# aloe101/GNOT-Replication

Measured on AMD Instinct MI355X. Metric: mesh points/sec (GNOT fwd+bwd, whole node), higher is better.
Workload: dtype fp32; 1 GPU; configs[2]: synthetic 3-D mesh of 262,144 points, d=256, 8 experts, 8 heads, 1 input function (805 points), fp32 fwd+bwd; samples_per_gpu=1, input_function_points=805, hidden=256, experts=8, heads=8, blocks=4, mlp_layers=4, input_functions=1, geometry=fixed, moe_recompute=False, parallelism=single, step=pack+fwd+RelL2+bwd+AdamW (native loss, native flat AdamW) (hipGraph replay)

## Files before the change

### gnot-replication_amd/csrc/engine.cpp

```cpp
#include <hip/hip_runtime.h>

#include <algorithm>
#include <cmath>
#include <cstdio>
#include <cstdlib>
#include <cstring>
#include <map>
#include <string>
#include <vector>

#include "../../include/gnot_hip.h"
#include "gnot_kernels.h"

namespace gnot {

static thread_local std::string g_err;

static int fail(int code, const std::string& msg) {
  g_err = msg;
  return code;
}

#define GNOT_CK(expr)                                                                           \
  do {                                                                                          \
// ... 487 lines not shown
      Img t = img(DT, DT);
      job(li, t, 0, 0, DT, DT, 1, -1, x6, li != io);
      p->T_img[li] = t;
    }
    if (!selftype)
      for (size_t i = 0; i < ik.size(); ++i)
        for (int li : {ik[i], iv[i]}) {
          Img t = new_img(DT, DT);
          job(li, t, 0, 0, DT, DT, 1, -1, 0, true);
          p->T_img[li] = t;
        }
  };
  for (int l = 0; l < p->L; ++l) {
    std::vector<int> ck, cv;
    for (int i = 0; i < p->KI; ++i) { ck.push_back(p->lin_ck(l, i)); cv.push_back(p->lin_cv(l, i)); }
    attn_imgs(p->cross_img[l], p->lin_cq(l), p->lin_co(l), ck, cv, p->I == 0);
    attn_imgs(p->self_img[l], p->lin_sq(l), p->lin_so(l), {p->lin_sk(l)}, {p->lin_sv(l)}, true);
    for (int e = 0; e < p->E; ++e) {
      chain_imgs(p->lin_f1(l, e, 0), DT, DT);
      chain_imgs(p->lin_f2(l, e, 0), DT, DT);
    }
  }
  chain_imgs(p->lin_out(0), DT, kt_of(p->out));
  p->pack_prefix.clear();
  int acc = 0;
  for (auto& J : p->pack_jobs) {
    p->pack_prefix.push_back(acc);
    acc += pack_tiles(J);
  }
  p->pack_tiles = acc;
}

constexpr long kWide128Wgs = 128;
static bool balanced_wgrad(const WgradGroup& G) {
  if (G.jobs.size() < 2) return false;
  for (const auto& J : G.jobs)
    if (J.P <= 0) return false;
  return 256 % (long)G.jobs.size() != 0;
}
static void finish_group(gnot_plan* p, WgradGroup& G) {
  G.x6 = true;
  for (const auto& J : G.jobs)
    if (J.w != nullptr || J.state_dh > 0 || J.diag_only) G.x6 = false;
  constexpr long x6_wgs = 256;
  const bool small = p->P < gnot_plan::kWgradSerialPoints;
  const long wide_wgs = !small ? 256 : p->npk() == 1 ? 64 : 128;
  const long w128_wgs = small && p->npk() != 1 ? 192 : kWide128Wgs;
  G.wide = G.x6 && p->D == 256 && !G.jobs.empty();
  for (const auto& J : G.jobs)
    if (J.out > 256 || J.in > 256) G.wide = false;
  G.tw = 256;
  if (G.x6 && !G.wide && p->D <= 128 && !G.jobs.empty()) {
    bool fits = true;
    for (const auto& J : G.jobs)
      if (J.out > 128 || J.in > 128) fits = false;
    if (fits) { G.wide = true; G.tw = 128; }
  }
  if (G.b16) G.wide = true;
  const long target = G.wide ? (G.tw == 128 ? w128_wgs : wide_wgs) : G.x6 ? x6_wgs : kTargetWGs;
  long tiles = 0;
  for (auto& J : G.jobs) {
    J.tiles_o = (J.out + kPTile - 1) / kPTile;
    J.tiles_i = (J.in + kPTile - 1) / kPTile;
    tiles += G.wide ? 1 : J.diag_only ? J.tiles_o : J.tiles_o * J.tiles_i;
  }
  const long want = std::max<long>(1, target / std::max<long>(tiles, 1));
  G.wg_prefix.clear();
  G.red_prefix.clear();
  G.segs.clear();
  G.seg_start.clear();
  G.slab_floats = 0;
  if (G.wide && G.tw == 256 && balanced_wgrad(G)) {
    long T = 0, maxrow = 1;
    for (const auto& J : G.jobs) {
      T += J.P;
      maxrow = std::max<long>(maxrow, G.b16 ? 512L : 4L * std::max<long>(std::max<long>(J.lddz, J.ldx), 1));
    }
    long C = std::max<long>((T + target - 1) / target, kMinSplitPoints);
    C = (C + 31) / 32 * 32;
    C = std::min<long>(C, ((1L << 31) - 1) / maxrow - 64);
    std::vector<long> jstart(G.jobs.size() + 1, 0);
    for (size_t j = 0; j < G.jobs.size(); ++j) jstart[j + 1] = jstart[j] + G.jobs[j].P;
    std::vector<int> nslots(G.jobs.size(), 0);
    size_t jj = 0;
    for (long w0 = 0; w0 < T; w0 += C) {
      const long w1 = std::min(T, w0 + C);
      G.seg_start.push_back((int)G.segs.size());
      while (jj < G.jobs.size() && jstart[jj + 1] <= w0) ++jj;
      for (size_t j = jj; j < G.jobs.size() && jstart[j] < w1; ++j) {
        const long b = std::max(w0, jstart[j]) - jstart[j], e = std::min(w1, jstart[j + 1]) - jstart[j];
        if (e > b) G.segs.push_back(int4{(int)j, nslots[j]++, (int)b, (int)e});
      }
    }
    G.seg_start.push_back((int)G.segs.size());
    int red = 0;
    for (size_t j = 0; j < G.jobs.size(); ++j) {
      auto& J = G.jobs[j];
      J.splits = std::max(1, nslots[j]);
      const int nt = J.tiles_o * J.tiles_i;
      J.slab_off = (long)G.slab_floats;
      G.slab_floats += (size_t)J.splits * nt * kPTile * (kPTile + 1);
      G.wg_prefix.push_back(0);
      G.red_prefix.push_back(red);
      red += nt * kPTile * (kPTile + 1);
    }
// ... 1653 lines not shown
```

### gnot-replication_amd/csrc/microbench.cpp

```cpp
#include <hip/hip_runtime.h>

#include <cstdio>
#include <algorithm>
#include <cmath>
#include <cstdlib>
#include <vector>

#include "gnot_kernels.h"

using namespace gnot;
#ifdef GNOT_DIAG_STAMP
namespace gnot {
hipError_t set_chain2_diag(int v);
}
#endif

#define CK(x)                                                                                   \
  do {                                                                                          \
    hipError_t e_ = (x);                                                                        \
    if (e_ != hipSuccess) {                                                                     \
      std::fprintf(stderr, "%s:%d %s -> %s\n", __FILE__, __LINE__, #x, hipGetErrorString(e_)); \
      std::exit(1);                                                                             \
    }                                                                                           \
  } while (0)

static float* dalloc(size_t n, float scale) {
  std::vector<float> h(n);
  for (size_t i = 0; i < n; ++i) h[i] = scale * ((float)((i * 2654435761u) % 2001) / 1000.0f - 1.0f);
  float* d = nullptr;
  CK(hipMalloc(&d, n * sizeof(float)));
  CK(hipMemcpy(d, h.data(), n * sizeof(float), hipMemcpyHostToDevice));
  return d;
}

template <typename F>
static double time_us(F&& f, int reps = 50) {
  hipEvent_t a, b;
  CK(hipEventCreate(&a));
  CK(hipEventCreate(&b));
  for (int i = 0; i < 5; ++i) f();
  CK(hipEventRecord(a, nullptr));
  for (int i = 0; i < reps; ++i) f();
  CK(hipEventRecord(b, nullptr));
  CK(hipEventSynchronize(b));
  float ms = 0.f;
  CK(hipEventElapsedTime(&ms, a, b));
  return ms * 1e3 / reps;
}

#ifdef GNOT_DIAG_STAMP
static void stamp_report(const char* name, ChainArgs a, bool bwd) {
  static unsigned long long* dbg = nullptr;
  const size_t n = (size_t)65536 * 8 * 3;
  if (!dbg) CK(hipMalloc(&dbg, n * sizeof(unsigned long long)));
  CK(hipMemset(dbg, 0, n * sizeof(unsigned long long)));
  a.dbg = dbg;
  CK(bwd ? launch_chain_bwd(a, nullptr) : launch_chain_fwd(a, nullptr));
  CK(hipDeviceSynchronize());
  std::vector<unsigned long long> h(n);
  CK(hipMemcpy(h.data(), dbg, n * sizeof(unsigned long long), hipMemcpyDeviceToHost));
  double body = 0, sync = 0, cnt = 0, waves = 0;
  for (size_t i = 0; i < n; i += 3)
    if (h[i + 2]) { body += (double)h[i]; sync += (double)h[i + 1]; cnt += (double)h[i + 2]; waves += 1; }
  std::printf("stamp %-28s waves %8.0f  syncs/wave %6.1f  sync share %5.3f  ticks/sync %7.1f  body ticks/interval %8.1f\n",
              name, waves, cnt / std::max(waves, 1.0), sync / std::max(body + sync, 1.0), sync / std::max(cnt, 1.0),
              body / std::max(cnt - waves, 1.0));
}
#define STAMP(name, args, bwd) stamp_report(name, args, bwd)
#else
#define STAMP(name, args, bwd) (void)0
#endif

int main(int argc, char** argv) {
  const int P = argc > 1 ? std::atoi(argv[1]) : 10000;
  const int D = argc > 2 ? std::atoi(argv[2]) : 128;
  const int E = argc > 3 ? std::atoi(argv[3]) : 4, NL = 5, DT = D / 16;
  const size_t img4 = (size_t)DT * ((DT + 1) / 2) * 3 * 64;
  float4* W = reinterpret_cast<float4*>(dalloc(img4 * 4 * NL * E * 2, 0.05f));
  float* bias = dalloc((size_t)NL * E * D, 0.01f);
  std::vector<ChainLayer> layers;
  for (int e = 0; e < E; ++e)
    for (int j = 0; j < NL; ++j) {
      const size_t k = (size_t)e * NL + j;
      layers.push_back(ChainLayer{W + 2 * k * img4, W + (2 * k + 1) * img4, bias + k * D});
    }
  ChainLayer* dlayers = nullptr;
  CK(hipMalloc(&dlayers, layers.size() * sizeof(ChainLayer)));
  CK(hipMemcpy(dlayers, layers.data(), layers.size() * sizeof(ChainLayer), hipMemcpyHostToDevice));
  float* X = dalloc((size_t)P * D, 1.0f);
  float* Y = dalloc((size_t)E * P * D, 0.0f);
  float* save = dalloc((size_t)E * NL * P * D, 1.0f);
  float* dz = dalloc((size_t)E * NL * P * D, 0.0f);
  float* scores = dalloc((size_t)P * 16, 0.25f);
  float* dscore = dalloc((size_t)P * 16, 0.0f);
  float* dX = dalloc((size_t)E * P * D, 0.0f);

  ChainArgs a{};
  a.D = D; a.KT0 = DT; a.OTL = DT; a.nlin = NL; a.in_dim = D; a.out_dim = D; a.P = P; a.nchains = E;
  a.layers = dlayers; a.X = X; a.ldx = D; a.Y = Y; a.ldy = D; a.y_chain_stride = (long)P * D;
  a.scores = scores; a.ldsc = 16; a.mode = CH_MOE;
  a.save = save; a.save_layer_stride = (long)P * D; a.save_chain_stride = (long)NL * P * D;
  const double fl = 2.0 * E * P * NL * (double)D * D;
  double t = time_us([&] { CK(launch_moe_combine(X, Y, (long)P * D, E, dX, (long)P * D, nullptr)); });
  std::printf("moe_combine E=%d P=%d D=%d: %8.2f us  %6.0f GB/s\n", E, P, D, t, (E + 2.0) * P * D * 4 / t / 1e3);
  t = time_us([&] { CK(launch_chain_fwd(a, nullptr)); });
  std::printf("chain_fwd  MoE E=%d P=%d D=%d: %8.2f us  %6.1f TFLOP/s\n", E, P, D, t, fl / t / 1e6);
  STAMP("chain_fwd MoE x6", a, false);
  {
    ChainArgs an = a;
    an.save = nullptr;
    t = time_us([&] { CK(launch_chain_fwd(an, nullptr)); });
    std::printf("chain_fwd  MoE no-save E=%d P=%d D=%d: %8.2f us  %6.1f TFLOP/s\n", E, P, D, t, fl / t / 1e6);
  }
  ChainArgs bw = a;
  bw.dY = X; bw.lddy = D; bw.dscore = dscore; bw.dz = dz; bw.dz_layer_stride = (long)P * D;
  bw.dz_chain_stride = (long)NL * P * D; bw.dX = dX; bw.lddx = D; bw.dx_chain_stride = (long)P * D;
  t = time_us([&] { CK(launch_chain_bwd(bw, nullptr)); });
  std::printf("chain_bwd  MoE E=%d P=%d D=%d: %8.2f us  %6.1f TFLOP/s\n", E, P, D, t, fl / t / 1e6);
  STAMP("chain_bwd MoE x6", bw, true);
  if (D == 256) {
    ChainArgs a1 = a, b1 = bw;
    a1.np = 1; b1.np = 1;
    t = time_us([&] { CK(launch_chain_fwd(a1, nullptr)); });
// ... 23 lines not shown
      t = time_us([&] { CK(launch_chain_bwd(bw, nullptr)); });
      std::printf("diag %d  fp32 (x6)    fwd %8.2f us  bwd %8.2f us\n", dg, tx, t);
    }
    CK(set_chain2_diag(0));
#else
    t = time_us([&] { CK(launch_chain_fwd(a3, nullptr)); });
    std::printf("chain_fwd  b16s stage E=%d P=%d D=%d: %8.2f us  %6.1f TFLOP/s\n", E, P, D, t, fl / t / 1e6);
    t = time_us([&] { CK(launch_chain_bwd(b3, nullptr)); });
    std::printf("chain_bwd  b16s stage E=%d P=%d D=%d: %8.2f us  %6.1f TFLOP/s\n", E, P, D, t, fl / t / 1e6);
#endif
  }

  if (argc > 4 && std::atoi(argv[4]) == 1) return 0;
  for (int NO : {D, 3 * D}) {
    LinearArgs l{};
    l.nseg = 1; l.X[0] = X; l.Wp[0] = W; l.ldx = D; l.nsum = 1; l.K = D; l.bias = bias; l.Y = Y; l.ldy = NO;
    l.NO = NO; l.P = P; l.epi = EPI_STORE; l.nsoft = 0; l.dh = 16;
    t = time_us([&] { CK(D == 256 ? launch_linear2(l, nullptr) : launch_linear(l, D, nullptr)); });
    std::printf("linear     P=%d K=%d NO=%d: %8.2f us  %6.1f TFLOP/s\n", P, D, NO, t, 2.0 * P * D * NO / t / 1e6);
    if (D == 256) {
      l.np = 1;
      t = time_us([&] { CK(launch_linear2(l, nullptr)); });
      std::printf("linear     P=%d K=%d NO=%d bf16: %8.2f us  %6.1f TFLOP/s\n", P, D, NO, t, 2.0 * P * D * NO / t / 1e6);
      l.np = 3;
    }
    if (D == 256 && NO == D) {
      l.epi = EPI_ACCUM;
      t = time_us([&] { CK(launch_linear2(l, nullptr)); });
      std::printf("linear     P=%d K=%d NO=%d accum: %8.2f us  %6.1f TFLOP/s\n", P, D, NO, t, 2.0 * P * D * NO / t / 1e6);
      l.nseg = 3; l.X[1] = X; l.X[2] = X; l.Wp[1] = W; l.Wp[2] = W; l.bias = nullptr;
      t = time_us([&] { CK(launch_linear2(l, nullptr)); });
      std::printf("linear     P=%d K=3x%d NO=%d accum: %8.2f us  %6.1f TFLOP/s\n", P, D, NO, t, 6.0 * P * D * NO / t / 1e6);
    }
  }
  {
    float* fresh = dalloc((size_t)E * NL * P * D, 0.5f);
    CK(hipMemcpy(dz, fresh, (size_t)E * NL * P * D * 4, hipMemcpyDeviceToDevice));
    CK(hipFree(fresh));
    fresh = dalloc((size_t)E * NL * P * D, 2.0f);
    CK(hipMemcpy(save, fresh, (size_t)E * NL * P * D * 4, hipMemcpyDeviceToDevice));
    CK(hipFree(fresh));
  }
  {
    std::vector<WgradJob> jobs;
    std::vector<int> wg_pre, red_pre;
    int wg = 0, red = 0;
    long slab_off = 0;
    float* dW = dalloc((size_t)E * NL * (D * D + D), 0.f);
    const int njobs = E * NL;
    const int tiles = ((D + 127) / 128) * ((D + 127) / 128);
    const long want = std::max<long>(1, 512 / ((long)njobs * tiles));
    for (int k = 0; k < njobs; ++k) {
      WgradJob J{};
      J.dz = dz + (size_t)k * P * D; J.lddz = D; J.x = save + (size_t)k * P * D; J.ldx = D; J.x_gelu = 1;
      J.out = D; J.in = D; J.dW = dW + (size_t)k * (D * D + D); J.db = J.dW + D * D; J.P = P;
      J.tiles_o = (D + 127) / 128; J.tiles_i = J.tiles_o;
      J.splits = (int)std::min<long>(std::min<long>(want, std::max<long>(1, P / 128)), 256);
      J.slab_off = slab_off;
      slab_off += (long)J.splits * tiles * 128 * 129;
      wg_pre.push_back(wg); wg += tiles * J.splits;
      red_pre.push_back(red); red += tiles * 128 * 129;
      jobs.push_back(J);
    }
    WgradJob* djobs = nullptr;
    int* dpre = nullptr;
    CK(hipMalloc(&djobs, jobs.size() * sizeof(WgradJob)));
// ... 14 lines not shown
    CK(hipMemcpy(got.data(), dW, ndw * 4, hipMemcpyDeviceToHost));
    double num = 0, den = 0;
    for (size_t i = 0; i < ndw; ++i) { num += (got[i] - ref[i]) * (double)(got[i] - ref[i]); den += (double)ref[i] * ref[i]; }
    std::printf("wgrad MoE  bf16x6:                     %8.2f us  %6.1f TFLOP/s  (rel-L2 vs fp32 %.2e)\n", t, fl / t / 1e6,
                std::sqrt(num / (den + 1e-30)));
    if (D == 256) {
      for (int wgs : {256, 512}) {
        std::vector<WgradJob> wj(jobs);
        std::vector<int> wpre;
        long soff = 0;
        const int splits = std::max(1, wgs / njobs);
        for (int k = 0; k < njobs; ++k) {
          wj[k].splits = splits;
          wj[k].slab_off = soff;
          soff += (long)splits * tiles * 128 * 129;
          wpre.push_back(k * splits);
        }
        wpre.insert(wpre.end(), red_pre.begin(), red_pre.end());
        WgradJob* dwj = nullptr;
        int* dwpre = nullptr;
        float* wslab = nullptr;
        CK(hipMalloc(&dwj, wj.size() * sizeof(WgradJob)));
        CK(hipMemcpy(dwj, wj.data(), wj.size() * sizeof(WgradJob), hipMemcpyHostToDevice));
        CK(hipMalloc(&dwpre, wpre.size() * sizeof(int)));
        CK(hipMemcpy(dwpre, wpre.data(), wpre.size() * sizeof(int), hipMemcpyHostToDevice));
        CK(hipMalloc(&wslab, soff * sizeof(float)));
        t = time_us([&] { CK(launch_wgrad(dwj, dwpre, njobs, njobs * splits, dwpre + njobs, red, wslab, nullptr, true, true)); }, 20);
        CK(hipDeviceSynchronize());
        CK(hipMemcpy(got.data(), dW, ndw * 4, hipMemcpyDeviceToHost));
        double n2 = 0, d2 = 0;
        for (size_t i = 0; i < ndw; ++i) { n2 += (got[i] - ref[i]) * (double)(got[i] - ref[i]); d2 += (double)ref[i] * ref[i]; }
        std::printf("wgrad MoE  bf16x6 wide 256x256 (%d WGs):  %8.2f us  %6.1f TFLOP/s  (rel-L2 vs fp32 %.2e)\n",
                    njobs * splits, t, fl / t / 1e6, std::sqrt(n2 / (d2 + 1e-30)));
        t = time_us([&] { CK(launch_wgrad(dwj, dwpre, njobs, njobs * splits, dwpre + njobs, red, wslab, nullptr, true, true, 1)); }, 20);
        CK(hipDeviceSynchronize());
        CK(hipMemcpy(got.data(), dW, ndw * 4, hipMemcpyDeviceToHost));
        n2 = 0; d2 = 0;
        for (size_t i = 0; i < ndw; ++i) { n2 += (got[i] - ref[i]) * (double)(got[i] - ref[i]); d2 += (double)ref[i] * ref[i]; }
        std::printf("wgrad MoE  bf16 wide 256x256 (%d WGs):    %8.2f us  %6.1f TFLOP/s  (rel-L2 vs fp32 %.2e)\n",
                    njobs * splits, t, fl / t / 1e6, std::sqrt(n2 / (d2 + 1e-30)));
        if (wgs == 512) {
          const char* what[3] = {"no-GELU operand", "L2-resident rows", "no-GELU + L2 rows"};
          for (int v = 0; v < 3; ++v) {
            std::vector<WgradJob> dj(wj);
            for (auto& J : dj) {
              if (v != 1) J.x_gelu = 0;
              if (v != 0) { J.lddz = 0; J.ldx = 0; }
            }
            CK(hipMemcpy(dwj, dj.data(), dj.size() * sizeof(WgradJob), hipMemcpyHostToDevice));
            t = time_us([&] { CK(launch_wgrad(dwj, dwpre, njobs, njobs * splits, dwpre + njobs, red, wslab, nullptr, true, true)); }, 20);
            std::printf("wgrad MoE  bf16x6 wide, %-18s   %8.2f us  %6.1f TFLOP/s\n", what[v], t, fl / t / 1e6);
          }
        }
        CK(hipFree(dwj));
        CK(hipFree(dwpre));
        CK(hipFree(wslab));
      }
    }
    {
      std::vector<WgradJob> ng(jobs);
      for (auto& J : ng) J.x_gelu = 0;
      WgradJob* dng = nullptr;
      CK(hipMalloc(&dng, ng.size() * sizeof(WgradJob)));
      CK(hipMemcpy(dng, ng.data(), ng.size() * sizeof(WgradJob), hipMemcpyHostToDevice));
      t = time_us([&] { CK(launch_wgrad(dng, dpre, njobs, wg, dpre + njobs, red, slab, nullptr)); }, 20);
      std::printf("wgrad MoE  no-GELU operand:            %8.2f us  %6.1f TFLOP/s\n", t, fl / t / 1e6);
// ... 55 lines not shown
```

### gnot-replication_amd/csrc/wgrad.hip

```cpp
#include <cstdlib>
#include <type_traits>

#include "gnot_common.h"
#include "gnot_kernels.h"
#include "x6_core.h"

namespace gnot {

typedef float f32x16 __attribute__((ext_vector_type(16)));

constexpr int kTile = 128;
constexpr int kStage = 32;
constexpr int kLdsRow = kTile;

GNOT_DEV int find_job(const int* __restrict__ prefix, int njobs, int idx) {
  int lo = 0, hi = njobs - 1;
  while (lo < hi) {
    const int mid = (lo + hi + 1) >> 1;
    if (prefix[mid] <= idx) lo = mid; else hi = mid - 1;
  }
  return lo;
}

struct StageRegs {
// ... 265 lines not shown
      asm volatile("" ::: "memory");
    }
  }

  const int ntile = J.tiles_o * J.tiles_i;
  const int tile = to * J.tiles_i + ti;
  float* S = slab + J.slab_off + ((long)split * ntile + tile) * (kTile * (kTile + 1));
#pragma unroll
  for (int a = 0; a < 2; ++a)
#pragma unroll
    for (int b = 0; b < 2; ++b)
#pragma unroll
      for (int r = 0; r < 16; ++r) {
        const int row = wo * 64 + a * 32 + (r & 3) + 8 * (r >> 2) + 4 * h;
        const int col = wi * 64 + b * 32 + r32;
        S[row * (kTile + 1) + col] = acc[a][b][r];
      }
  if (want_db) {
    __syncthreads();
    float* red = reinterpret_cast<float*>(lds);
    red[o * kTile + 2 * fp] = dbacc[0];
    red[o * kTile + 2 * fp + 1] = dbacc[1];
    __syncthreads();
    if (tid < kTile) S[tid * (kTile + 1) + kTile] = (red[tid] + red[kTile + tid]) + (red[2 * kTile + tid] + red[3 * kTile + tid]);
  }
}

constexpr int kWStage = 16;
constexpr int kWThreads = 512;
constexpr int w_threads(int tw) { return tw * 2; }
constexpr int w_piece(int tw) { return tw / 32 * 64; }
constexpr int w_buf(int np, int tw = 256) { return 2 * np * w_piece(tw); }
constexpr int kWRawSlot = 2 * 2 * 64;
constexpr int kWRawSlots = 2;
constexpr size_t w_lds_bytes(int np, int tw = 256) {
  return (2 * (size_t)w_buf(np, tw) + (size_t)(tw / 32) * kWRawSlots * kWRawSlot) * 16;
}

template <int OFF>
GNOT_DEV float lds_read_b32_off(unsigned addr) {
  float v;
  asm volatile("ds_read_b32 %0, %1 offset:%2" : "=v"(v) : "v"(addr), "n"(OFF) : "memory");
  return v;
}

template <int NP = 3, int TW = 256>
__global__ void __launch_bounds__(w_threads(TW)) pgemm_x6w_kernel(const WgradJob* __restrict__ jobs,
                                                                 const int* __restrict__ prefix, int njobs,
                                                                 float* __restrict__ slab,
                                                                 const int4* __restrict__ segs,
                                                                 const int* __restrict__ seg_start) {
  constexpr int NW = TW / 32;
  constexpr int FG = TW / 64;
  constexpr int WC = NW / 2;
  constexpr int RB = TW / 64;
  constexpr int kWPiece = w_piece(TW);
  extern __shared__ __attribute__((aligned(16))) u32x4 wl[];
  const int tid = threadIdx.x;
  const int lane = tid & 63, wave = __builtin_amdgcn_readfirstlane(tid >> 6);
  int k0 = 0, k1 = 1;
  if (segs != nullptr) { k0 = seg_start[blockIdx.x]; k1 = seg_start[blockIdx.x + 1]; }
  for (int kseg = k0; kseg < k1; ++kseg) {
  int j, split;
  long pb, pe;
  if (segs != nullptr) {
    const int4 sg = segs[kseg];
    j = sg.x; split = sg.y; pb = sg.z; pe = sg.w;
    if (kseg > k0) __syncthreads();
  } else {
    j = find_job(prefix, njobs, blockIdx.x);
    split = blockIdx.x - prefix[j];
    const int chunk = ((jobs[j].P + jobs[j].splits - 1) / jobs[j].splits + kWStage - 1) / kWStage * kWStage;
    pb = (long)split * chunk;
    pe = min((long)jobs[j].P, pb + chunk);
  }
  const WgradJob J = jobs[j];
  const int nst = pe > pb ? (int)((pe - pb + kWStage - 1) / kWStage) : 0;
  const int f = tid & (TW - 1), hh = tid / TW;
  const bool fa = f < J.out, fb = f < J.in;
  const int sdst = (f >> 5) * 64 + (f & 31) + 32 * hh;
  const int wr = wave / WC, wc = wave % WC;
  const int nrb = max(0, min(RB, (J.out - 32 * RB * wr + 31) / 32));
  const int ncb = max(0, min(2, (J.in - 64 * wc + 31) / 32));
  const bool full = nrb == RB && ncb == 2;
  const bool gel = J.x_gelu != 0;

  f32x16 acc[RB][2];
#pragma unroll
  for (int a = 0; a < RB; ++a)
#pragma unroll
    for (int b = 0; b < 2; ++b) acc[a][b] = f32x16{};
  float dbacc = 0.f;
  float ra_raw[8], rb_raw[8];
  const long nsp = pe > pb ? pe - pb : 0;
  const rsrc_t rA = make_rsrc(J.dz + pb * J.lddz, (unsigned)(nsp * J.lddz * 4));
  const rsrc_t rB = make_rsrc(J.x + pb * J.ldx, (unsigned)(nsp * J.ldx * 4));
  const int fcol = 64 * (wave % FG) + 4 * (lane & 15);
  const int dvA = ((lane >> 4) * (int)J.lddz + fcol) * 4, dvB = ((lane >> 4) * (int)J.ldx + fcol) * 4;
  u32x4* const raw = wl + 2 * w_buf(NP, TW) + wave * kWRawSlots * kWRawSlot;
  auto raw_dma = [&](int st) __attribute__((always_inline)) {
    u32x4* dst = raw + (st & 1) * kWRawSlot;
    const unsigned p0 = (unsigned)(st * kWStage + 8 * (wave / FG));
#pragma unroll
    for (int i = 0; i < 2; ++i) {
      dma16(rA, dst + i * 64, dvA, (int)((p0 + 4 * i) * (unsigned)J.lddz * 4u));
      dma16(rB, dst + 128 + i * 64, dvB, (int)((p0 + 4 * i) * (unsigned)J.ldx * 4u));
    }
  };
  const unsigned raw_addr = (unsigned)(uintptr_t)(const __attribute__((address_space(3))) u32x4*)raw + 4u * lane;
  auto raw_read = [&](int st) __attribute__((always_inline)) {
    const unsigned a = raw_addr + (unsigned)((st & 1) * kWRawSlot * 16);
    ra_raw[0] = lds_read_b32_off<0>(a);    rb_raw[0] = lds_read_b32_off<2048>(a);
    ra_raw[1] = lds_read_b32_off<256>(a);  rb_raw[1] = lds_read_b32_off<2304>(a);
    ra_raw[2] = lds_read_b32_off<512>(a);  rb_raw[2] = lds_read_b32_off<2560>(a);
    ra_raw[3] = lds_read_b32_off<768>(a);  rb_raw[3] = lds_read_b32_off<2816>(a);
    ra_raw[4] = lds_read_b32_off<1024>(a); rb_raw[4] = lds_read_b32_off<3072>(a);
    ra_raw[5] = lds_read_b32_off<1280>(a); rb_raw[5] = lds_read_b32_off<3328>(a);
    ra_raw[6] = lds_read_b32_off<1536>(a); rb_raw[6] = lds_read_b32_off<3584>(a);
    ra_raw[7] = lds_read_b32_off<1792>(a); rb_raw[7] = lds_read_b32_off<3840>(a);
    asm volatile("s_waitcnt lgkmcnt(0)"
                 : "+v"(ra_raw[0]), "+v"(ra_raw[1]), "+v"(ra_raw[2]), "+v"(ra_raw[3]), "+v"(ra_raw[4]),
                   "+v"(ra_raw[5]), "+v"(ra_raw[6]), "+v"(ra_raw[7]), "+v"(rb_raw[0]), "+v"(rb_raw[1]),
                   "+v"(rb_raw[2]), "+v"(rb_raw[3]), "+v"(rb_raw[4]), "+v"(rb_raw[5]), "+v"(rb_raw[6]),
                   "+v"(rb_raw[7])::"memory");
  };
  auto stage_v = [&](int buf, auto GEL) {
    float ra[8], vb[8];
#pragma unroll
    for (int k = 0; k < 8; ++k) {
      ra[k] = fa ? ra_raw[k] : 0.f;
      const float b = fb ? rb_raw[k] : 0.f;
      dbacc += ra[k];
      vb[k] = decltype(GEL)::value ? gelu(b) : b;
    }
    u32x4 pa[NP], pq[NP];
    split8_np<NP>(ra, pa);
    split8_np<NP>(vb, pq);
    u32x4* base = wl + buf * w_buf(NP, TW);
#pragma unroll
    for (int q = 0; q < NP; ++q) {
      base[q * kWPiece + sdst] = pa[q];
      base[(NP + q) * kWPiece + sdst] = pq[q];
    }
  };
  auto stage = [&](int buf) {
    if (gel) stage_v(buf, std::true_type{});
    else stage_v(buf, std::false_type{});
  };
  auto compute = [&](int buf) {
    const u32x4* A = wl + buf * w_buf(NP, TW);
    const u32x4* Bm = A + NP * kWPiece;
    u32x4 bf[2][NP];
#pragma unroll
    for (int jb = 0; jb < 2; ++jb)
#pragma unroll
      for (int q = 0; q < NP; ++q) bf[jb][q] = Bm[q * kWPiece + (wc * 2 + jb) * 64 + lane];
#pragma unroll
    for (int ib = 0; ib < RB; ++ib) {
      if (ib >= nrb) break;
      u32x4 af[NP];
#pragma unroll
      for (int q = 0; q < NP; ++q) af[q] = A[q * kWPiece + (wr * RB + ib) * 64 + lane];
      if (ncb > 0) mfma_np<NP>(af, bf[0], acc[ib][0]);
      if (ncb > 1) mfma_np<NP>(af, bf[1], acc[ib][1]);
    }
  };
  auto lds_barrier = []() __attribute__((always_inline)) { asm volatile("s_waitcnt lgkmcnt(0)\n\ts_barrier" ::: "memory"); };

  if (nst > 0) {
    raw_dma(0);
    raw_dma(1);
    c2_wait_vm<4>();
    raw_read(0);
    raw_dma(2);
    stage(0);
    lds_barrier();
    int buf = 0;
    auto fused = [&](int b, auto GEL, auto MASK) {
      const u32x4* A = wl + b * w_buf(NP, TW);
      const u32x4* Bm = A + NP * kWPiece;
      u32x4 bf[2][NP], af[2][NP], pa[NP], pq[NP];
#pragma unroll
      for (int jb = 0; jb < 2; ++jb)
#pragma unroll
        for (int q = 0; q < NP; ++q) bf[jb][q] = Bm[q * kWPiece + (wc * 2 + jb) * 64 + lane];
#pragma unroll
      for (int q = 0; q < NP; ++q) af[0][q] = A[q * kWPiece + (wr * RB) * 64 + lane];
      float ra[8], vb[8];
      auto chunk = [&](int k) {
        ra[k] = (!decltype(MASK)::value || fa) ? ra_raw[k] : 0.f;
        dbacc += ra[k];
        const float bv = (!decltype(MASK)::value || fb) ? rb_raw[k] : 0.f;
        vb[k] = decltype(GEL)::value ? gelu(bv) : bv;
        asm volatile("" : "+v"(ra[k]), "+v"(vb[k]), "+v"(dbacc));
        if (k & 1) {
          split2_np<NP>(ra[k - 1], ra[k], pa, k >> 1);
          split2_np<NP>(vb[k - 1], vb[k], pq, k >> 1);
#pragma unroll
          for (int q = 0; q < NP; ++q) asm volatile("" : "+v"(pa[q][k >> 1]), "+v"(pq[q][k >> 1]));
        }
      };
      constexpr int CPG = 8 / (2 * RB);
#pragma unroll
      for (int ib = 0; ib < RB; ++ib) {
        if (ib + 1 < RB) {
#pragma unroll
          for (int q = 0; q < NP; ++q) af[(ib + 1) & 1][q] = A[q * kWPiece + (wr * RB + ib + 1) * 64 + lane];
        }
        mfma_np<NP>(af[ib & 1], bf[0], acc[ib][0]);
        __builtin_amdgcn_sched_barrier(0);
#pragma unroll
        for (int k = 0; k < CPG; ++k) chunk(CPG * 2 * ib + k);
        __builtin_amdgcn_sched_barrier(0);
        mfma_np<NP>(af[ib & 1], bf[1], acc[ib][1]);
        __builtin_amdgcn_sched_barrier(0);
#pragma unroll
        for (int k = 0; k < CPG; ++k) chunk(CPG * (2 * ib + 1) + k);
        __builtin_amdgcn_sched_barrier(0);
      }
      u32x4* base = wl + (b ^ 1) * w_buf(NP, TW);
#pragma unroll
      for (int q = 0; q < NP; ++q) {
        base[q * kWPiece + sdst] = pa[q];
        base[(NP + q) * kWPiece + sdst] = pq[q];
      }
    };
    auto run = [&](auto GEL, auto MASK) {
      for (int s = 0; s + 1 < nst; ++s) {
        c2_wait_vm<4>();
        raw_read(s + 1);
        raw_dma(s + 3);
        fused(buf, GEL, MASK);
        lds_barrier();
        buf ^= 1;
      }
    };
    if (full) {
      if (J.out >= TW && J.in >= TW) {
        if (gel) run(std::true_type{}, std::false_type{});
        else run(std::false_type{}, std::false_type{});
      } else {
        if (gel) run(std::true_type{}, std::true_type{});
        else run(std::false_type{}, std::true_type{});
      }
    } else {
      for (int s = 0; s + 1 < nst; ++s) {
        c2_wait_vm<4>();
        raw_read(s + 1);
        raw_dma(s + 3);
        compute(buf);
        stage(buf ^ 1);
        lds_barrier();
        buf ^= 1;
      }
    }
    compute(buf);
    asm volatile("s_waitcnt vmcnt(0)" ::: "memory");
  }

  const int ntile = J.tiles_o * J.tiles_i;
  float* S0 = slab + J.slab_off + (long)split * ntile * (kTile * (kTile + 1));
#pragma unroll
  for (int ib = 0; ib < RB; ++ib)
#pragma unroll
    for (int jb = 0; jb < 2; ++jb)
#pragma unroll
      for (int r = 0; r < 16; ++r) {
        const int row = wr * 32 * RB + ib * 32 + (r & 3) + 8 * (r >> 2) + 4 * (lane >> 5);
        const int col = wc * 64 + jb * 32 + (lane & 31);
        if (row < J.out && col < J.in)
          S0[((row >> 7) * J.tiles_i + (col >> 7)) * (kTile * (kTile + 1)) + (row & 127) * (kTile + 1) + (col & 127)] =
              acc[ib][jb][r];
      }
  if (J.db != nullptr) {
    float* red = reinterpret_cast<float*>(wl);
    __syncthreads();
    red[hh * TW + f] = dbacc;
    __syncthreads();
    if (tid < TW && f < J.out)
      S0[((f >> 7) * J.tiles_i) * (kTile * (kTile + 1)) + (f & 127) * (kTile + 1) + kTile] = red[f] + red[TW + f];
  }
  }
}

constexpr int kBStage = 32;
constexpr int kBSlots = 4;
constexpr int kBOpnd = kBStage * kB16Row;
constexpr int kBSlotBytes = 2 * kBOpnd;
constexpr size_t kBLds = (size_t)kBSlots * kBSlotBytes;

GNOT_DEV u32x2 lds_tr_b64(unsigned addr) {
  u32x2 v;
  asm volatile("ds_read_b64_tr_b16 %0, %1" : "=v"(v) : "v"(addr) : "memory");
  return v;
}

__global__ void __launch_bounds__(kWThreads) pgemm_b16_kernel(const WgradJob* __restrict__ jobs,
                                                             const int* __restrict__ prefix, int njobs,
                                                             float* __restrict__ slab, const int4* __restrict__ segs,
                                                             const int* __restrict__ seg_start) {
  extern __shared__ __attribute__((aligned(16))) u32x4 bl[];
  const int tid = threadIdx.x, lane = tid & 63;
  const int wave = __builtin_amdgcn_readfirstlane(tid >> 6);
  int k0 = 0, k1 = 1;
  if (segs != nullptr) { k0 = seg_start[blockIdx.x]; k1 = seg_start[blockIdx.x + 1]; }
  for (int kseg = k0; kseg < k1; ++kseg) {
  int j, split;
  long pb, pe;
  if (segs != nullptr) {
    const int4 sg = segs[kseg];
    j = sg.x; split = sg.y; pb = sg.z; pe = sg.w;
    if (kseg > k0) __syncthreads();
  } else {
    j = find_job(prefix, njobs, blockIdx.x);
    split = blockIdx.x - prefix[j];
// ... 125 lines not shown
  for (; k + 8 <= J.splits; k += 8)
#pragma unroll
    for (int u = 0; u < 8; ++u) part[u] += S[(long)(k + u) * sstride];
  for (; k < J.splits; ++k) part[0] += S[(long)k * sstride];
  const float s = ((part[0] + part[1]) + (part[2] + part[3])) + ((part[4] + part[5]) + (part[6] + part[7]));
  float* dst;
  if (J.state_dh > 0) {
    const int dh = J.state_dh, hh = row / dh, i = row % dh;
    float* base = J.dW + (long)hh * (dh * dh + dh);
    dst = isdb ? base + dh * dh + i : base + i * dh + (col % dh);
  } else {
    dst = isdb ? (J.db + row) : (J.dW + (long)row * J.in + col);
  }
  *dst = (accumulate && J.state_dh == 0) ? (*dst + s) : s;
}

hipError_t launch_wgrad_b16(const WgradJob* jobs_dev, const int* wg_prefix_dev, int njobs, int total_wgs,
                            const int* red_prefix_dev, int total_red, float* slab, hipStream_t s, const int4* segs,
                            const int* seg_start, bool accumulate) {
  if (njobs <= 0) return hipSuccess;
  static bool attr = false;
  if (!attr) {
    (void)hipFuncSetAttribute(reinterpret_cast<const void*>(pgemm_b16_kernel), hipFuncAttributeMaxDynamicSharedMemorySize,
                              (int)kBLds);
    attr = true;
  }
  hipLaunchKernelGGL(pgemm_b16_kernel, dim3(total_wgs), dim3(kWThreads), kBLds, s, jobs_dev, wg_prefix_dev, njobs, slab,
                     segs, seg_start);
  hipLaunchKernelGGL(pgemm_reduce_kernel, dim3((total_red + 255) / 256), dim3(256), 0, s, jobs_dev, red_prefix_dev,
                     njobs, total_red, (const float*)slab, accumulate ? 1 : 0);
  return hipGetLastError();
}

hipError_t launch_wgrad(const WgradJob* jobs_dev, const int* wg_prefix_dev, int njobs, int total_wgs,
                        const int* red_prefix_dev, int total_red, float* slab, hipStream_t s, bool x6, bool wide,
                        int np, int tw, const int4* segs, const int* seg_start, bool accumulate) {
  if (njobs <= 0) return hipSuccess;
  if (wide) {
    const size_t lds = w_lds_bytes(np, tw);
#define GNOT_X6W(NP_, TW_)                                                                                     \
  if (np == NP_ && tw == TW_) {                                                                                \
    static bool attr = false;                                                                                  \
    if (!attr) {                                                                                               \
      (void)hipFuncSetAttribute(reinterpret_cast<const void*>(pgemm_x6w_kernel<NP_, TW_>),                     \
                                hipFuncAttributeMaxDynamicSharedMemorySize, (int)lds);                         \
      attr = true;                                                                                             \
    }                                                                                                          \
    hipLaunchKernelGGL((pgemm_x6w_kernel<NP_, TW_>), dim3(total_wgs), dim3(w_threads(TW_)), lds, s, jobs_dev,  \
                       wg_prefix_dev, njobs, slab, segs, seg_start);                                           \
  }
    GNOT_X6W(3, 256) GNOT_X6W(1, 256) GNOT_X6W(3, 128) GNOT_X6W(1, 128)
#undef GNOT_X6W
  } else if (x6) {
    if (np == 1) hipLaunchKernelGGL(pgemm_x6_kernel<1>, dim3(total_wgs), dim3(256), 0, s, jobs_dev, wg_prefix_dev, njobs, slab);
    else hipLaunchKernelGGL(pgemm_x6_kernel<3>, dim3(total_wgs), dim3(256), 0, s, jobs_dev, wg_prefix_dev, njobs, slab);
  }
  else
    hipLaunchKernelGGL(pgemm_kernel, dim3(total_wgs), dim3(256), 0, s, jobs_dev, wg_prefix_dev, njobs, slab);
  hipLaunchKernelGGL(pgemm_reduce_kernel, dim3((total_red + 255) / 256), dim3(256), 0, s, jobs_dev,
                     red_prefix_dev, njobs, total_red, (const float*)slab, accumulate ? 1 : 0);
  return hipGetLastError();
}

}
```

Measured before the change: 1.077 million points/s.

## Single-buffer wgrad fragments with early stores for wide NP=3 kernel

The wide 256-column bf16x6 weight-gradient kernel, for NP=3, now keeps one fragment buffer in LDS instead of two. It writes the next stage's fragments during the last row block, after a mid-loop barrier. This frees LDS, which may allow more workgroups per CU, and moves the stores earlier so they overlap MFMA work. The cost is an extra barrier per stage. The balanced-split heuristic now checks divisibility against the real workgroup target instead of a fixed 256, and diagnostic timing variants are added to the microbenchmark.

After: 1.084 million points/s, median of 6. Within noise of the previous version (+0.7%).

```diff
diff --git a/gnot-replication_amd/csrc/engine.cpp b/gnot-replication_amd/csrc/engine.cpp
--- a/gnot-replication_amd/csrc/engine.cpp
+++ b/gnot-replication_amd/csrc/engine.cpp
@@ -543,11 +543,11 @@
 }
 
 constexpr long kWide128Wgs = 128;
-static bool balanced_wgrad(const WgradGroup& G) {
+static bool balanced_wgrad(const WgradGroup& G, long target) {
   if (G.jobs.size() < 2) return false;
   for (const auto& J : G.jobs)
     if (J.P <= 0) return false;
-  return 256 % (long)G.jobs.size() != 0;
+  return target % (long)G.jobs.size() != 0;
 }
 static void finish_group(gnot_plan* p, WgradGroup& G) {
   G.x6 = true;
@@ -581,7 +581,7 @@
   G.segs.clear();
   G.seg_start.clear();
   G.slab_floats = 0;
-  if (G.wide && G.tw == 256 && balanced_wgrad(G)) {
+  if (G.wide && G.tw == 256 && balanced_wgrad(G, target)) {
     long T = 0, maxrow = 1;
     for (const auto& J : G.jobs) {
       T += J.P;
diff --git a/gnot-replication_amd/csrc/microbench.cpp b/gnot-replication_amd/csrc/microbench.cpp
--- a/gnot-replication_amd/csrc/microbench.cpp
+++ b/gnot-replication_amd/csrc/microbench.cpp
@@ -4,16 +4,23 @@
 #include <algorithm>
 #include <cmath>
 #include <cstdlib>
+#include <cstring>
 #include <vector>
 
 #include "gnot_kernels.h"
 
 using namespace gnot;
+#if defined(GNOT_DIAG_STAMP) && !defined(GNOT_WGRAD_FORMS)
+#define GNOT_WGRAD_FORMS
+#endif
+namespace gnot {
 #ifdef GNOT_DIAG_STAMP
-namespace gnot {
 hipError_t set_chain2_diag(int v);
-}
-#endif
+#endif
+#ifdef GNOT_WGRAD_FORMS
+hipError_t set_wgrad_diag(int form, unsigned long long* dbg);
+#endif
+}
 
 #define CK(x)                                                                                   \
   do {                                                                                          \
@@ -67,6 +74,27 @@
               body / std::max(cnt - waves, 1.0));
 }
 #define STAMP(name, args, bwd) stamp_report(name, args, bwd)
+template <typename F>
+static void wgrad_stamp_report(const char* name, int form, int waves, F&& launch) {
+  static unsigned long long* dbg = nullptr;
+  const size_t n = (size_t)4096 * 8 * 6;
+  if ((size_t)waves * 6 > n) return;
+  if (!dbg) CK(hipMalloc(&dbg, n * sizeof(unsigned long long)));
+  CK(hipMemset(dbg, 0, n * sizeof(unsigned long long)));
+  CK(set_wgrad_diag(form, dbg));
+  launch();
+  CK(hipDeviceSynchronize());
+  std::vector<unsigned long long> h((size_t)waves * 6);
+  CK(hipMemcpy(h.data(), dbg, h.size() * sizeof(unsigned long long), hipMemcpyDeviceToHost));
+  double s[6] = {0, 0, 0, 0, 0, 0};
+  for (int w = 0; w < waves; ++w)
+    for (int i = 0; i < 6; ++i) s[i] += (double)h[(size_t)w * 6 + i];
+  const double loop = std::max(s[4], 1.0), it = std::max(s[5], 1.0);
+  std::printf("stamp wgrad %-38s waves %5d  iters/wave %7.1f  ticks/iter %7.1f  shares: vmcnt wait %5.3f  raw read %5.3f  "
+              "end barrier %5.3f  mid barrier %5.3f\n",
+              name, waves, s[5] / waves, s[4] / it, s[0] / loop, s[1] / loop, s[2] / loop, s[3] / loop);
+  CK(set_wgrad_diag(form, nullptr));
+}
 #else
 #define STAMP(name, args, bwd) (void)0
 #endif
@@ -88,7 +116,7 @@
   CK(hipMalloc(&dlayers, layers.size() * sizeof(ChainLayer)));
   CK(hipMemcpy(dlayers, layers.data(), layers.size() * sizeof(ChainLayer), hipMemcpyHostToDevice));
   float* X = dalloc((size_t)P * D, 1.0f);
-  float* Y = dalloc((size_t)E * P * D, 0.0f);
+  float* Y = dalloc((size_t)std::max(E, 3) * P * D, 0.0f);
   float* save = dalloc((size_t)E * NL * P * D, 1.0f);
   float* dz = dalloc((size_t)E * NL * P * D, 0.0f);
   float* scores = dalloc((size_t)P * 16, 0.25f);
@@ -178,6 +206,10 @@
       t = time_us([&] { CK(launch_linear2(l, nullptr)); });
       std::printf("linear     P=%d K=3x%d NO=%d accum: %8.2f us  %6.1f TFLOP/s\n", P, D, NO, t, 6.0 * P * D * NO / t / 1e6);
     }
+  }
+  if (argc > 4 && std::atoi(argv[4]) == 2) {
+    CK(hipDeviceSynchronize());
+    return 0;
   }
   {
     float* fresh = dalloc((size_t)E * NL * P * D, 0.5f);
@@ -258,6 +290,27 @@
         for (size_t i = 0; i < ndw; ++i) { n2 += (got[i] - ref[i]) * (double)(got[i] - ref[i]); d2 += (double)ref[i] * ref[i]; }
         std::printf("wgrad MoE  bf16x6 wide 256x256 (%d WGs):  %8.2f us  %6.1f TFLOP/s  (rel-L2 vs fp32 %.2e)\n",
                     njobs * splits, t, fl / t / 1e6, std::sqrt(n2 / (d2 + 1e-30)));
+#ifdef GNOT_WGRAD_FORMS
+        if (wgs == 256) {
+          const char* fname[5] = {"shipped", "ring 2, 2 buffers, late stores (r06)", "ring 2, 2 buffers, early stores",
+                                  "ring 2, 1 buffer", "ring 3, 1 buffer"};
+          auto once = [&] { CK(launch_wgrad(dwj, dwpre, njobs, njobs * splits, dwpre + njobs, red, wslab, nullptr, true, true)); };
+          std::vector<float> alt(ndw);
+          for (int form : {1, 2, 3, 4, 0, 1, 2, 3, 4, 0}) {
+#ifdef GNOT_DIAG_STAMP
+            wgrad_stamp_report(fname[form], form, njobs * splits * 8, once);
+#else
+            CK(set_wgrad_diag(form, nullptr));
+#endif
+            t = time_us(once, 20);
+            CK(hipDeviceSynchronize());
+            CK(hipMemcpy(alt.data(), dW, ndw * 4, hipMemcpyDeviceToHost));
+            std::printf("form  wgrad %-38s %8.2f us  bitwise == shipped: %s\n", fname[form], t,
+                        std::memcmp(alt.data(), got.data(), ndw * 4) == 0 ? "yes" : "NO");
+          }
+          CK(set_wgrad_diag(0, nullptr));
+        }
+#endif
         t = time_us([&] { CK(launch_wgrad(dwj, dwpre, njobs, njobs * splits, dwpre + njobs, red, wslab, nullptr, true, true, 1)); }, 20);
         CK(hipDeviceSynchronize());
         CK(hipMemcpy(got.data(), dW, ndw * 4, hipMemcpyDeviceToHost));
diff --git a/gnot-replication_amd/csrc/wgrad.hip b/gnot-replication_amd/csrc/wgrad.hip
--- a/gnot-replication_amd/csrc/wgrad.hip
+++ b/gnot-replication_amd/csrc/wgrad.hip
@@ -321,10 +321,21 @@
 constexpr int w_piece(int tw) { return tw / 32 * 64; }
 constexpr int w_buf(int np, int tw = 256) { return 2 * np * w_piece(tw); }
 constexpr int kWRawSlot = 2 * 2 * 64;
-constexpr int kWRawSlots = 2;
-constexpr size_t w_lds_bytes(int np, int tw = 256) {
-  return (2 * (size_t)w_buf(np, tw) + (size_t)(tw / 32) * kWRawSlots * kWRawSlot) * 16;
-}
+constexpr int w_ring(int np, int tw) { return 2; }
+constexpr int w_nbuf(int np, int tw) { return tw == 256 && np == 3 ? 1 : 2; }
+constexpr bool w_early(int np, int tw) { return tw == 256 && np == 3; }
+constexpr size_t w_lds_bytes(int np, int tw, int k, int nb) {
+  return ((size_t)nb * w_buf(np, tw) + (size_t)(tw / 32) * k * kWRawSlot) * 16;
+}
+#if defined(GNOT_DIAG_STAMP) && !defined(GNOT_WGRAD_FORMS)
+#define GNOT_WGRAD_FORMS
+#endif
+#ifdef GNOT_DIAG_STAMP
+__device__ unsigned long long* g_wgrad_dbg = nullptr;
+#define GNOT_WST(...) __VA_ARGS__
+#else
+#define GNOT_WST(...)
+#endif
 
 template <int OFF>
 GNOT_DEV float lds_read_b32_off(unsigned addr) {
@@ -333,12 +344,15 @@
   return v;
 }
 
-template <int NP = 3, int TW = 256>
+template <int NP = 3, int TW = 256, int K = w_ring(NP, TW), int NB = w_nbuf(NP, TW), bool ES = w_early(NP, TW)>
 __global__ void __launch_bounds__(w_threads(TW)) pgemm_x6w_kernel(const WgradJob* __restrict__ jobs,
                                                                  const int* __restrict__ prefix, int njobs,
                                                                  float* __restrict__ slab,
                                                                  const int4* __restrict__ segs,
                                                                  const int* __restrict__ seg_start) {
+  static_assert(K >= 2 && (K + 1) * kWStage <= 64, "finish_group leaves 64 rows of offset room past a range's end");
+  static_assert(!ES || TW == 256, "early stores: the staging fits the first RB - 1 row blocks only at RB = 4");
+  static_assert(NB == 2 || (NB == 1 && ES), "one fragment buffer is overwritten during the last row block");
   constexpr int NW = TW / 32;
   constexpr int FG = TW / 64;
   constexpr int WC = NW / 2;
@@ -349,6 +363,7 @@
   const int lane = tid & 63, wave = __builtin_amdgcn_readfirstlane(tid >> 6);
   int k0 = 0, k1 = 1;
   if (segs != nullptr) { k0 = seg_start[blockIdx.x]; k1 = seg_start[blockIdx.x + 1]; }
+  GNOT_WST(unsigned long long ts_vm = 0, ts_rd = 0, ts_bar = 0, ts_mid = 0, ts_loop = 0, ts_n = 0;)
   for (int kseg = k0; kseg < k1; ++kseg) {
   int j, split;
   long pb, pe;
@@ -386,9 +401,9 @@
   const rsrc_t rB = make_rsrc(J.x + pb * J.ldx, (unsigned)(nsp * J.ldx * 4));
   const int fcol = 64 * (wave % FG) + 4 * (lane & 15);
   const int dvA = ((lane >> 4) * (int)J.lddz + fcol) * 4, dvB = ((lane >> 4) * (int)J.ldx + fcol) * 4;
-  u32x4* const raw = wl + 2 * w_buf(NP, TW) + wave * kWRawSlots * kWRawSlot;
-  auto raw_dma = [&](int st) __attribute__((always_inline)) {
-    u32x4* dst = raw + (st & 1) * kWRawSlot;
+  u32x4* const raw = wl + NB * w_buf(NP, TW) + wave * K * kWRawSlot;
+  auto raw_dma = [&](int st, int slot) __attribute__((always_inline)) {
+    u32x4* dst = raw + slot * kWRawSlot;
     const unsigned p0 = (unsigned)(st * kWStage + 8 * (wave / FG));
 #pragma unroll
     for (int i = 0; i < 2; ++i) {
@@ -397,8 +412,8 @@
     }
   };
   const unsigned raw_addr = (unsigned)(uintptr_t)(const __attribute__((address_space(3))) u32x4*)raw + 4u * lane;
-  auto raw_read = [&](int st) __attribute__((always_inline)) {
-    const unsigned a = raw_addr + (unsigned)((st & 1) * kWRawSlot * 16);
+  auto raw_read = [&](int slot) __attribute__((always_inline)) {
+    const unsigned a = raw_addr + (unsigned)(slot * kWRawSlot * 16);
     ra_raw[0] = lds_read_b32_off<0>(a);    rb_raw[0] = lds_read_b32_off<2048>(a);
     ra_raw[1] = lds_read_b32_off<256>(a);  rb_raw[1] = lds_read_b32_off<2304>(a);
     ra_raw[2] = lds_read_b32_off<512>(a);  rb_raw[2] = lds_read_b32_off<2560>(a);
@@ -455,16 +470,27 @@
     }
   };
   auto lds_barrier = []() __attribute__((always_inline)) { asm volatile("s_waitcnt lgkmcnt(0)\n\ts_barrier" ::: "memory"); };
+#ifdef GNOT_DIAG_STAMP
+  auto lds_barrier_st = [&](unsigned long long& sum) __attribute__((always_inline)) {
+    const unsigned long long t0 = c2_stamp();
+    lds_barrier();
+    sum += c2_stamp() - t0;
+  };
+#define GNOT_WBAR(sum) lds_barrier_st(sum)
+#else
+#define GNOT_WBAR(sum) lds_barrier()
+#endif
 
   if (nst > 0) {
-    raw_dma(0);
-    raw_dma(1);
-    c2_wait_vm<4>();
+#pragma unroll
+    for (int st = 0; st < K; ++st) raw_dma(st, st);
+    c2_wait_vm<4 * (K - 1)>();
     raw_read(0);
-    raw_dma(2);
+    raw_dma(K, 0);
     stage(0);
     lds_barrier();
     int buf = 0;
+    int rs = 1;
     auto fused = [&](int b, auto GEL, auto MASK) {
       const u32x4* A = wl + b * w_buf(NP, TW);
       const u32x4* Bm = A + NP * kWPiece;
@@ -489,40 +515,60 @@
           for (int q = 0; q < NP; ++q) asm volatile("" : "+v"(pa[q][k >> 1]), "+v"(pq[q][k >> 1]));
         }
       };
-      constexpr int CPG = 8 / (2 * RB);
+      constexpr int NG = ES ? 2 * (RB - 1) : 2 * RB;
+      auto chunks = [&](int g) {
+#pragma unroll
+        for (int k = 8 * g / NG; k < 8 * (g + 1) / NG; ++k) chunk(k);
+      };
+      auto store_pieces = [&](u32x4* base) {
+#pragma unroll
+        for (int q = 0; q < NP; ++q) {
+          base[q * kWPiece + sdst] = pa[q];
+          base[(NP + q) * kWPiece + sdst] = pq[q];
+        }
+      };
 #pragma unroll
       for (int ib = 0; ib < RB; ++ib) {
         if (ib + 1 < RB) {
 #pragma unroll
           for (int q = 0; q < NP; ++q) af[(ib + 1) & 1][q] = A[q * kWPiece + (wr * RB + ib + 1) * 64 + lane];
+        }
+        const bool lastb = ES && ib == RB - 1;
+        if (NB == 1 && lastb) {
+          __builtin_amdgcn_sched_barrier(0);
+          GNOT_WBAR(ts_mid);
+          __builtin_amdgcn_sched_barrier(0);
         }
         mfma_np<NP>(af[ib & 1], bf[0], acc[ib][0]);
         __builtin_amdgcn_sched_barrier(0);
-#pragma unroll
-        for (int k = 0; k < CPG; ++k) chunk(CPG * 2 * ib + k);
+        if (lastb) store_pieces(wl + (NB == 1 ? 0 : (b ^ 1) * w_buf(NP, TW)));
+        else chunks(2 * ib);
         __builtin_amdgcn_sched_barrier(0);
         mfma_np<NP>(af[ib & 1], bf[1], acc[ib][1]);
         __builtin_amdgcn_sched_barrier(0);
-#pragma unroll
-        for (int k = 0; k < CPG; ++k) chunk(CPG * (2 * ib + 1) + k);
+        if (!lastb) chunks(2 * ib + 1);
         __builtin_amdgcn_sched_barrier(0);
       }
-      u32x4* base = wl + (b ^ 1) * w_buf(NP, TW);
-#pragma unroll
-      for (int q = 0; q < NP; ++q) {
-        base[q * kWPiece + sdst] = pa[q];
-        base[(NP + q) * kWPiece + sdst] = pq[q];
-      }
+      if constexpr (!ES) store_pieces(wl + (b ^ 1) * w_buf(NP, TW));
+    };
+    auto next_rows = [&](int s) __attribute__((always_inline)) {
+      GNOT_WST(const unsigned long long t0 = c2_stamp();)
+      c2_wait_vm<4 * (K - 1)>();
+      GNOT_WST(const unsigned long long t1 = c2_stamp();)
+      raw_read(rs);
+      GNOT_WST(const unsigned long long t2 = c2_stamp(); ts_vm += t1 - t0; ts_rd += t2 - t1; ++ts_n;)
+      raw_dma(s + K + 1, rs);
+      rs = rs + 1 == K ? 0 : rs + 1;
     };
     auto run = [&](auto GEL, auto MASK) {
+      GNOT_WST(const unsigned long long tb = c2_stamp();)
       for (int s = 0; s + 1 < nst; ++s) {
-        c2_wait_vm<4>();
-        raw_read(s + 1);
-        raw_dma(s + 3);
+        next_rows(s);
         fused(buf, GEL, MASK);
-        lds_barrier();
-        buf ^= 1;
-      }
+        GNOT_WBAR(ts_bar);
+        if constexpr (NB == 2) buf ^= 1;
+      }
+      GNOT_WST(ts_loop += c2_stamp() - tb;)
     };
     if (full) {
       if (J.out >= TW && J.in >= TW) {
@@ -534,13 +580,16 @@
       }
     } else {
       for (int s = 0; s + 1 < nst; ++s) {
-        c2_wait_vm<4>();
-        raw_read(s + 1);
-        raw_dma(s + 3);
+        next_rows(s);
         compute(buf);
-        stage(buf ^ 1);
+        if constexpr (NB == 1) {
+          lds_barrier();
+          stage(buf);
+        } else {
+          stage(buf ^ 1);
+          buf ^= 1;
+        }
         lds_barrier();
-        buf ^= 1;
       }
     }
     compute(buf);
@@ -570,6 +619,13 @@
       S0[((f >> 7) * J.tiles_i) * (kTile * (kTile + 1)) + (f & 127) * (kTile + 1) + kTile] = red[f] + red[TW + f];
   }
   }
+#undef GNOT_WBAR
+#ifdef GNOT_DIAG_STAMP
+  if (g_wgrad_dbg != nullptr && lane == 0) {
+    unsigned long long* d = g_wgrad_dbg + ((size_t)blockIdx.x * NW + wave) * 6;
+    d[0] = ts_vm; d[1] = ts_rd; d[2] = ts_bar; d[3] = ts_mid; d[4] = ts_loop; d[5] = ts_n;
+  }
+#endif
 }
 
 constexpr int kBStage = 32;
@@ -761,25 +817,48 @@
   return hipGetLastError();
 }
 
+#ifdef GNOT_WGRAD_FORMS
+static int g_wgrad_form = 0;
+hipError_t set_wgrad_diag(int form, unsigned long long* dbg) {
+  g_wgrad_form = form;
+#ifdef GNOT_DIAG_STAMP
+  return hipMemcpyToSymbol(HIP_SYMBOL(g_wgrad_dbg), &dbg, sizeof(dbg));
+#else
+  return dbg == nullptr ? hipSuccess : hipErrorInvalidValue;
+#endif
+}
+#endif
+
 hipError_t launch_wgrad(const WgradJob* jobs_dev, const int* wg_prefix_dev, int njobs, int total_wgs,
                         const int* red_prefix_dev, int total_red, float* slab, hipStream_t s, bool x6, bool wide,
                         int np, int tw, const int4* segs, const int* seg_start, bool accumulate) {
   if (njobs <= 0) return hipSuccess;
   if (wide) {
-    const size_t lds = w_lds_bytes(np, tw);
-#define GNOT_X6W(NP_, TW_)                                                                                     \
-  if (np == NP_ && tw == TW_) {                                                                                \
+#define GNOT_X6W_FORM(NP_, TW_, K_, NB_, ES_)                                                                  \
+  {                                                                                                            \
+    constexpr size_t lds = w_lds_bytes(NP_, TW_, K_, NB_);                                                     \
+    static_assert(lds <= 160 * 1024, "one CU's LDS");                                                          \
     static bool attr = false;                                                                                  \
     if (!attr) {                                                                                               \
-      (void)hipFuncSetAttribute(reinterpret_cast<const void*>(pgemm_x6w_kernel<NP_, TW_>),                     \
+      (void)hipFuncSetAttribute(reinterpret_cast<const void*>(pgemm_x6w_kernel<NP_, TW_, K_, NB_, ES_>),       \
                                 hipFuncAttributeMaxDynamicSharedMemorySize, (int)lds);                         \
       attr = true;                                                                                             \
     }                                                                                                          \
-    hipLaunchKernelGGL((pgemm_x6w_kernel<NP_, TW_>), dim3(total_wgs), dim3(w_threads(TW_)), lds, s, jobs_dev,  \
-                       wg_prefix_dev, njobs, slab, segs, seg_start);                                           \
-  }
+    hipLaunchKernelGGL((pgemm_x6w_kernel<NP_, TW_, K_, NB_, ES_>), dim3(total_wgs), dim3(w_threads(TW_)), lds, \
+                       s, jobs_dev, wg_prefix_dev, njobs, slab, segs, seg_start);                              \
+  }
+#define GNOT_X6W(NP_, TW_) \
+  if (np == NP_ && tw == TW_) GNOT_X6W_FORM(NP_, TW_, w_ring(NP_, TW_), w_nbuf(NP_, TW_), w_early(NP_, TW_))
+#ifdef GNOT_WGRAD_FORMS
+    if (np == 3 && tw == 256 && g_wgrad_form == 1) GNOT_X6W_FORM(3, 256, 2, 2, false)
+    else if (np == 3 && tw == 256 && g_wgrad_form == 2) GNOT_X6W_FORM(3, 256, 2, 2, true)
+    else if (np == 3 && tw == 256 && g_wgrad_form == 3) GNOT_X6W_FORM(3, 256, 2, 1, true)
+    else if (np == 3 && tw == 256 && g_wgrad_form == 4) GNOT_X6W_FORM(3, 256, 3, 1, true)
+    else
+#endif
     GNOT_X6W(3, 256) GNOT_X6W(1, 256) GNOT_X6W(3, 128) GNOT_X6W(1, 128)
 #undef GNOT_X6W
+#undef GNOT_X6W_FORM
   } else if (x6) {
     if (np == 1) hipLaunchKernelGGL(pgemm_x6_kernel<1>, dim3(total_wgs), dim3(256), 0, s, jobs_dev, wg_prefix_dev, njobs, slab);
     else hipLaunchKernelGGL(pgemm_x6_kernel<3>, dim3(total_wgs), dim3(256), 0, s, jobs_dev, wg_prefix_dev, njobs, slab);
```
